# melspectrum007/audio-visual-speech-enhancement

Hardware: AMD Instinct MI355X
Metric: clips/sec (STFT+CNN forward) on 200-ms@16kHz segments, 1/2/4/8 MI355X (higher is better)
Workload: dtype fp32_split

## Files before the change

### audio-visual-speech-enhancement_amd/csrc/avse_common.h

```cpp
#pragma once
#include <hip/hip_runtime.h>
#include <stdint.h>
#include <string>

#include "forward_plan.h"
#include "ragged_geom.h"

typedef __bf16 bf16_t;
typedef __bf16 bf16x8 __attribute__((ext_vector_type(8)));
typedef _Float16 f16x8 __attribute__((ext_vector_type(8)));
typedef _Float16 f16x4 __attribute__((ext_vector_type(4)));
typedef float f32x4 __attribute__((ext_vector_type(4)));
typedef int i32x4 __attribute__((ext_vector_type(4)));

struct avse_ctx;

namespace avse {

void set_error(const std::string& msg);

int ctx_device_index(const struct ::avse_ctx* c);

int ensure_lds_attr(const void* fn, int bytes);

// ... 154 lines not shown
constexpr int kConvSplit = 2, kConvSplitPairs = 3;
int launch_conv(const ConvArgs& a, int dtype, hipStream_t s);

int launch_conv_win(const ConvArgs& a, const int2* htaps, hipStream_t s);

struct DecTailArgs {
    const bf16_t* in;
    float* out;
    int N;
    const bf16_t* w4;
    const float* sc4;
    const float* sh4;
    int nt4, kpad4;
    int pt4, pl4, rows4, pitch4;
    int dy4, dx4, nx4;
    const bf16_t* w5;
    const float* sc5;
    const float* sh5;
    int nt5[4], kpad5[4];
    int dy5[4], dx5[4], nx5[4];
    long long woff5[4];
    int pt5, pl5, rows5, pitch5;
    const float* w6;
    float b6;
    unsigned* range_flag;
    unsigned range_bit;
    int four_products;
};
bool dec_tail_supported(const DecTailArgs& a);
bool dec_tail_s16_supported(const DecTailArgs& a);
int launch_dec_tail_s16(const DecTailArgs& a, hipStream_t s);

struct AudEncArgs {
    const float* mel;
    bf16_t* out;
    long long out_clip_stride;
    int N;
    const bf16_t* w1;
    const bf16_t* w2;
    const bf16_t* w3;
    const bf16_t* w4;
    const bf16_t* w5;
    const float* sc[5];
    const float* sh[5];
};
bool aud_enc_supported(const AudEncArgs& a);

struct DecHeadArgs {
    const bf16_t* in;
    long long in_clip_stride;
    bf16_t* out;
    long long out_clip_stride;
    int N;
    const bf16_t* w1;
    const bf16_t* w2;
    const bf16_t* w3;
    const float* sc[3];
    const float* sh[3];
};
bool dec_head_supported(const DecHeadArgs& a);
int launch_dec_head(const DecHeadArgs& a, hipStream_t s);

struct GemmArgs {
    const bf16_t* a;
    long long lda;
    const bf16_t* w;
    int M, N, kpad;
    const float* scale;
    const float* shift;
    int act;
    bf16_t* out;
    long long ldo;
    int out_off;
    int ksplit;
    float* partial;
    int* counters;
    int split;
    int slabs_per_split;
    unsigned* range_flag;
    unsigned range_bit;
    int counters_cap;
    int four_products;
};
int launch_gemm(const GemmArgs& g, int mode, hipStream_t s);
int launch_aud_enc(const AudEncArgs& a, hipStream_t s);
int launch_dec_tail(const DecTailArgs& a, hipStream_t s);

enum HaloOut { OUT_BF16 = 0, OUT_S16 = 1, OUT_F32 = 2 };

struct HaloArgs {
    int variant;
    const void* in;
    const float* video;
    const float* vmean;
    const float* vstd;
    void* out;
    const void* w;
    const float* scale;
    const float* shift;
    int N, Hc, Wc, Ci, Co;
    long long out_clip_stride;
    int out_pix_stride;
    int out_c_off;
    int mfma32;
    int no_planar;
    int split;
    int out_mode;
    unsigned long long* prof;
    unsigned* range_flag;
    unsigned range_bit, range_in_bit;
    int video_u8;
};

int launch_conv_stream(const HaloArgs& a, hipStream_t s);
int launch_conv_v1r(const HaloArgs& a, hipStream_t s);
int launch_video_prep(const void* video, int video_u8, const float* mean, const float* stdv, void* out, int64_t N,
                      int F, int dtype, hipStream_t s);
int launch_audio_prep(const float* audio, void* out, int64_t npix, int dtype, hipStream_t s);
int launch_aconv1_split(const float* in, const float* w, const float* scale, const float* shift, void* out, int64_t N,
                        int H, int W, int Ho, int Wo, int KH, int KW, int S, int pt, int pl, int Co, unsigned* range_flag,
                        unsigned range_bit, unsigned range_in_bit, hipStream_t s);
int launch_out_conv(const void* in, const float* w64, float bias, float* out, int64_t npix, int dtype,
                    hipStream_t s);
int launch_broadcast_row(const void* src, void* dst, int64_t rows, int64_t row_bytes, int64_t stride_bytes,
                         hipStream_t s);
int launch_video_normalize(float* video, int64_t S, int H, int W, int F, const float* mean,
                           const float* stdv, hipStream_t s);
int launch_mse(const float* a, const float* b, int64_t n, float* loss, float* partial, hipStream_t s);

size_t mix_pairs_scratch_bytes(int64_t n_pairs);
int launch_mix_pairs(const int16_t* speech, const int64_t* speech_off, const int16_t* noise, const int64_t* noise_off,
                     const double* snr_lin, int64_t n_pairs, int64_t L, float* rows, double* mix64, double* factor,
                     void* scratch, hipStream_t s);
constexpr int kVideoStatsMaxF = 8;
size_t video_stats_scratch_bytes(int64_t S, int H, int W);
int launch_video_stats(const float* video, int64_t S, int H, int W, int F, float* mean, float* stdv, void* scratch,
                       hipStream_t s);
int launch_video_stats_u8(const uint8_t* video, int64_t S, int H, int W, int F, float* mean, float* stdv, void* scratch,
                          hipStream_t s);

struct EvalDev {
    const double* taps;
    const double* W;
    const double* twid;
    const double* segw;
    const int* bands;
    int up, down, H;
    int win, skip;
    int stoi;
    int64_t cap;
    const double* ptaps;
    int ms;
};
size_t eval_pairs_scratch_bytes(int64_t n_pairs, const EvalDev& t);
int launch_eval_pairs(const float* ref, const float* deg, const int64_t* off, int64_t n_pairs, const EvalDev& t,
                      double* metrics, void* scratch, hipStream_t s);

}
```

### audio-visual-speech-enhancement_amd/csrc/capi.hip

```cpp
#include <algorithm>
#include <cmath>
#include <cstdlib>
#include <cstring>
#include <mutex>
#include <set>

#include "ctx.h"
#include "eval_tables.h"
#include "spec_tables.h"

namespace avse {
static thread_local std::string g_err;
void set_error(const std::string& msg) { g_err = msg; }

int ensure_lds_attr(const void* fn, int bytes) {
    static std::mutex mu;
    static std::set<std::pair<const void*, int>> done;
    int dev = 0;
    AVSE_HIP_CHECK(hipGetDevice(&dev));
    std::lock_guard<std::mutex> lock(mu);
    if (done.count({fn, dev})) return 0;
    AVSE_HIP_CHECK(hipFuncSetAttribute(fn, hipFuncAttributeMaxDynamicSharedMemorySize, bytes));
    done.insert({fn, dev});
    return 0;
}

int fail(int code, const std::string& msg) {
    set_error(msg);
    return code;
}

int ctx_device_index(const avse_ctx* c) { return c->device; }
}

using namespace avse;

static_assert(sizeof(Cplx) == sizeof(float2) && offsetof(Cplx, im) == offsetof(float2, y), "Cplx must match float2");
static_assert(sizeof(MelBin) == sizeof(float4) && offsetof(MelBin, j0) == offsetof(float4, z), "MelBin must match float4");

struct OptionName {
    const char* name;
    const char* env;
    int Options::*field;
};
const OptionName kOptionNames[] = {
    {"no_gemm", "AVSE_NO_GEMM", &Options::no_gemm},
    {"no_audenc", "AVSE_NO_AUDENC", &Options::no_audenc},
    {"no_dechead", "AVSE_NO_DECHEAD", &Options::no_dechead},
    {"no_dectail", "AVSE_NO_DECTAIL", &Options::no_dectail},
    {"unfused_tail", "AVSE_UNFUSED_TAIL", &Options::unfused_tail},
    {"no_halo", "AVSE_NO_HALO", &Options::no_halo},
    {"mfma32", "AVSE_MFMA32", &Options::mfma32},
    {"serial", "AVSE_SERIAL", &Options::serial},
    {"graph", "AVSE_GRAPH", &Options::graph},
    {"gemm_ksplit_cap", "AVSE_GEMM_KSPLIT", &Options::gemm_ksplit_cap},
    {"dense_istft", "AVSE_DENSE_ISTFT", &Options::dense_istft},
    {"no_act_scale", "AVSE_NO_ACT_SCALE", &Options::no_act_scale},
    {"no_win", "AVSE_NO_WIN", &Options::no_win},
    {"no_v1p", "AVSE_NO_V1P", &Options::no_v1p},
    {"no_a1valu", "AVSE_NO_A1VALU", &Options::no_a1valu},
    {"no_planar", "AVSE_NO_PLANAR", &Options::no_planar},
    {"four_products", "AVSE_FOUR_PRODUCTS", &Options::four_products},
    {"side_prio", "AVSE_SIDE_PRIO", &Options::side_prio},
};

namespace {

const OptionName* find_option(const char* name) {
    for (const OptionName& o : kOptionNames)
        if (std::strcmp(o.name, name) == 0) return &o;
    return nullptr;
}

int upload_ragged(avse_ctx* c, const RaggedGeom& g, hipStream_t s, RaggedDev* d) {
    const size_t ub = sizeof(RaggedUtt) * g.utt.size(), ib = sizeof(RaggedItem) * g.items.size();
    const size_t need = ub + ib;
    hipStreamCaptureStatus cs = hipStreamCaptureStatusNone;
    if (s) AVSE_HIP_CHECK(hipStreamIsCapturing(s, &cs));
    const bool capturing = cs != hipStreamCaptureStatusNone;
    if (int rc = grow(c->prep, need, s, "preprocess scratch")) return rc;
    if (!capturing && c->ragged_done) AVSE_HIP_CHECK(hipEventSynchronize(c->ragged_done));
    if (int rc = grow(c->ragged_host, need, s, "ragged tables")) return rc;
    if (!c->ragged_done) AVSE_HIP_CHECK(hipEventCreateWithFlags(&c->ragged_done, hipEventDisableTiming));
    std::memcpy(c->ragged_host, g.utt.data(), ub);
    std::memcpy(c->ragged_host + ub, g.items.data(), ib);
    AVSE_HIP_CHECK(hipMemcpyAsync(c->prep, c->ragged_host, need, hipMemcpyHostToDevice, s));
    if (!capturing) AVSE_HIP_CHECK(hipEventRecord(c->ragged_done, s));
    d->utt = reinterpret_cast<const RaggedUtt*>(c->prep.p.get());
    d->items = reinterpret_cast<const RaggedItem*>(c->prep + ub);
    d->n_utt = (int)g.utt.size();
    d->n_items = (int)g.items.size();
    return 0;
}

template <typename D, typename T>
int table_to_device(const std::vector<T>& h, Owned<D>& out) {
    static_assert(sizeof(D) == sizeof(T), "element layout");
    AVSE_HIP_CHECK(out.alloc(sizeof(T) * h.size()));
    AVSE_HIP_CHECK(hipMemcpy(out, h.data(), sizeof(T) * h.size(), hipMemcpyHostToDevice));
    return 0;
}

int ensure_spec_tables(avse_ctx* c, int sr, int n_fft, int n_mels, double fmin, double fmax) {
    return build_spec_tables(c->spec, sr, n_fft, n_mels, fmin, fmax);
}

int ensure_istft_tables(avse_ctx* c, int sr, int n_fft, int n_mels, double fmin, double fmax) {
    return build_istft_tables(c->istft, sr, n_fft, n_mels, fmin, fmax);
}

int ensure_eval_tables(avse_ctx* c, int sr, bool any_rate, hipStream_t s, const EvalTables** out) {
    int up, down;
    eval_ratio(sr, &up, &down);
    const bool big = any_rate && std::max(up, down) > kEvalMaxRatio;
    for (const EvalTables& have : c->eval)
        if (have.sr == sr && have.big == big) {
            *out = &have;
            return 0;
        }
    if (int rc = not_capturing(s, "the tables of this sample rate would be built while the stream is being captured: run "
                                  "one call with this rate before the capture"))
        return rc;
    EvalTables& t = c->eval[c->eval_next];
    c->eval_next = (c->eval_next + 1) % 4;
    *out = &t;
    t = EvalTables();
    const int win = seg_snr_window(sr);
    const bool stoi = big || std::max(up, down) <= kEvalMaxRatio;
    const std::vector<double> taps = stoi ? resample_taps(up, down) : resample_taps(1, 1);
    if (big) {
        if (int rc = table_to_device(resample_taps_by_phase(taps, up), t.ptaps)) return rc;
    } else {
        if (int rc = table_to_device(taps, t.taps)) return rc;
    }
    if (int rc = table_to_device(hann_inner(kStoiFrame), t.W)) return rc;
    if (int rc = table_to_device(stoi_twiddle(), t.twid)) return rc;
    if (int rc = table_to_device(hann_inner(win), t.segw)) return rc;
    if (int rc = table_to_device(stoi_bands(), t.bands)) return rc;
    t.up = up; t.down = down; t.H = ((int)taps.size() - 1) / 2; t.win = win;
    t.sr = sr;
    t.big = big;
    return 0;
}

int spec_check(bool pointers, int64_t n_utt, const int64_t* n_samples, int sr, int n_fft, int hop, int n_mels, int pad_mode,
// ... 380 lines not shown
```

### audio-visual-speech-enhancement_amd/csrc/forward.hip

```cpp
#include <algorithm>
#include <cstdio>
#include <cstring>

#include "ctx.h"

using namespace avse;

namespace {

HaloArgs halo_args(const GpuLayer& G, const void* in, const void* video, int video_dtype, const float* vmean,
                   const float* vstd, void* out, long long out_clip_stride, int out_pix_stride, int out_c_off, int64_t N,
                   const Options& opt) {
    HaloArgs a;
    std::memset(&a, 0, sizeof(a));
    a.variant = G.halo;
    a.in = in;
    a.video = reinterpret_cast<const float*>(video);
    a.video_u8 = video_dtype == AVSE_VIDEO_U8;
    a.vmean = vmean;
    a.vstd = vstd;
    a.out = out;
    a.w = G.w_halo;
    a.mfma32 = opt.mfma32;
    a.no_planar = opt.no_planar;
// ... 90 lines not shown
    a.Wq = G.wq;
    a.sy = (L.kind == CONV) ? L.sh : 1;
    a.sx = (L.kind == CONV) ? L.sw : 1;
    a.oys = (L.kind == DECONV) ? L.sh : 1;
    a.oxs = (L.kind == DECONV) ? L.sw : 1;
    a.Ho = G.ho;
    a.Wo = G.wo;
    a.Co = L.cout;
    a.out_clip_stride = out_clip_stride;
    a.out_pix_stride = out_pix_stride;
    a.out_c_off = out_c_off;
    a.pool = L.pool ? 1 : 0;
    a.act = 1;
    a.nphase = G.nphase;
    a.ksplit = 1;
    for (int p = 0; p < G.nphase; ++p) a.ph[p] = G.ph[p];
    return a;
}

int ensure_arena(avse_ctx* c, int64_t clips, int dtype, const ArenaShape& a, hipStream_t s) {
    const size_t need = std::max(arena_bytes(clips, dtype, c->opt, nullptr, a), arena_bytes(1, dtype, c->opt, nullptr, a));
    return grow(c->arena, need, s, "forward scratch", "call avse_ctx_reserve_weights(ctx, weights, max_clips) before the capture");
}

struct Run {
    avse_ctx* c;
    const avse_weights* W;
    const Options& opt;
    const NetPlan& P;
    hipStream_t s;
    hipEvent_t* ev;
    const int dt;
    const bool split;
    const int gdt;
    const int cdt;
    const bool use_gemm;
    int stage = 0;

    Run(avse_ctx* c_, const avse_weights* W_, hipStream_t s_, hipEvent_t* ev_)
        : c(c_), W(W_), opt(c_->opt), P(W_->shape.plan), s(s_), ev(ev_), dt(W_->dtype), split(dt == AVSE_F32_SPLIT),
          gdt(dt == AVSE_BF16 ? AVSE_BF16 : AVSE_F32), cdt(split ? kConvSplit : gdt),
          use_gemm((dt == AVSE_BF16 || split) && !opt.no_gemm) {}

    const GpuLayer& L(int i) const { return W->layers[i]; }
    size_t es() const { return dt == AVSE_BF16 ? 2 : 4; }

    int mark() {
        if (ev) AVSE_HIP_CHECK(hipEventRecord(ev[stage], s));
        ++stage;
        return 0;
    }
    int mark(int n) {
        for (int k = 0; k < n; ++k)
            if (int rc = mark()) return rc;
        return 0;
    }

    int pairs(ConvArgs& a, bool in_pairs, bool out_pairs, int li, unsigned* rflag) const {
        if (!split) return gdt;
        a.range_flag = rflag;
        a.range_bit = 1u << li;
        a.range_in_bit = li == 0 ? kRangeAudioIn : kRangeVideoIn;
        if (in_pairs) {
            a.Ci *= 2;
            a.in_clip_stride *= 2;
            for (int p = 0; p < a.nphase; ++p) {
                a.ph[p].kpad *= 2;
                a.ph[p].w_off *= 2;
            }
        }
        if (out_pairs) {
            a.out_s16 = 1;
            a.out_clip_stride *= 2;
            a.out_pix_stride *= 2;
            a.out_c_off *= 2;
        }
        return in_pairs ? kConvSplitPairs : kConvSplit;
    }

    int conv(const ConvArgs& a, int dti, const GpuLayer& G, hipStream_t st) const {
        if (split && dti == kConvSplitPairs && !opt.no_win) {
            const int rw = launch_conv_win(a, G.htaps, st);
            if (rw != -1) return rw;
        }
        return launch_conv(a, split ? dti : cdt, st);
    }

    int gemm_layer(int li, const void* in, long long lda, void* out, long long ldo, int out_pix_stride, int out_off,
                   int64_t n, size_t part_off, unsigned* rflag) const {
        const GpuLayer& G = L(li);
        const SplitPlan sp = split_plan(W->shape.split[li - kSplitFirst], n, dt, opt);
        float* partial = reinterpret_cast<float*>(c->arena + part_off);
        const int mode = li == kSplitFirst ? 1 : 0;
        if (use_gemm && (mode == 0 || W->v6_gemm_shape)) {
            GemmArgs g;
            std::memset(&g, 0, sizeof(g));
            g.a = reinterpret_cast<const bf16_t*>(in);
            g.w = reinterpret_cast<const bf16_t*>(G.w);
            g.out = reinterpret_cast<bf16_t*>(out);
            g.lda = split ? 2 * lda : lda;
            g.ldo = split ? 2 * ldo : ldo;
            g.out_off = split ? 2 * out_off : out_off;
            g.M = (int)(mode == 1 ? n * 16 : n); g.N = G.def.cout; g.kpad = G.ph[0].kpad;
            g.scale = G.scale; g.shift = G.shift; g.act = 1;
            g.ksplit = sp.gemm.ksplit; g.slabs_per_split = sp.gemm.slabs; g.partial = partial;
            g.counters = c->gemm_counters; g.counters_cap = kGemmCounters;
            g.split = split; g.four_products = opt.four_products;
            if (split) { g.range_flag = rflag; g.range_bit = 1u << li; }
            const int rc = launch_gemm(g, mode, s);
            if (rc != -1) return rc;
        }
        ConvArgs a = conv_args(G, in, lda, out, ldo, out_pix_stride, out_off, n);
        a.ksplit = sp.conv.ksplit; a.ksplit_slabs = sp.conv.slabs; a.partial = partial;
        const int dti = pairs(a, true, true, li, rflag);
        return launch_conv(a, split ? dti : cdt, s);
    }

    int video_encoder(const void* vid, int vid_dt, const float* vm, const float* vs, int64_t n, const size_t* o,
                      void* cat, unsigned* rflag, bool record) {
        const long long CAT = P.cat, AEMB = P.aemb;
        auto vb = [&](int b) { return (void*)(c->arena + o[b]); };
        const int v_in[6] = {B_VIN, B_V1, B_V2, B_V3, B_V4, B_V5};
        int rc;
        if (L(5).halo == HALO_NONE &&
            (rc = launch_video_prep(vid, vid_dt == AVSE_VIDEO_U8, vm, vs, vb(B_VIN), n, P.F, gdt, s)))
            return rc;
        for (int i = 0; i < 6; ++i) {
            const GpuLayer& G = L(5 + i);
            const long long in_cs = (long long)G.def.hin * G.def.win * (i == 0 ? G.cin_pad : G.def.cin);
            if (G.halo != HALO_NONE) {
                HaloArgs h = (i < 5) ? halo_args(G, vb(v_in[i]), vid, vid_dt, vm, vs, vb(v_in[i + 1]),
                                                 (long long)G.ho * G.wo * G.def.cout, G.def.cout, 0, n, opt)
                                     : halo_args(G, vb(v_in[i]), vid, vid_dt, vm, vs, cat, CAT, G.def.cout, AEMB, n, opt);
                if (split) {
                    h.split = 1;
                    h.range_flag = rflag;
                    h.range_bit = 1u << (5 + i);
                    h.range_in_bit = kRangeVideoIn;
                    if (G.halo != HALO_V1 && G.halo != HALO_V1P) h.Ci = 2 * G.def.cin;
                    h.out_mode = OUT_S16;
                    h.out_clip_stride *= 2;
                    h.out_pix_stride *= 2;
                    h.out_c_off *= 2;
                }
                rc = G.halo == HALO_V1 || G.halo == HALO_V1P ? launch_conv_v1r(h, s) : launch_conv_stream(h, s);
            } else if (i == 5) {
                rc = gemm_layer(5 + i, vb(v_in[i]), in_cs, cat, CAT, G.def.cout, AEMB, n, o[B_COUNT], rflag);
            } else {
                ConvArgs a = conv_args(G, vb(v_in[i]), in_cs, vb(v_in[i + 1]), (long long)G.ho * G.wo * G.def.cout, G.def.cout, 0, n);
                const int dti = pairs(a, i > 0, true, 5 + i, rflag);
                rc = launch_conv(a, split ? dti : cdt, s);
            }
            if (rc || (record && (rc = mark()))) return rc;
        }
        return 0;
    }

    int zero_video_embedding() {
        if (W->vzero_emb.load(std::memory_order_acquire)) return 0;
        std::lock_guard<std::mutex> lk(W->vzero_mu);
        if (W->vzero_emb.load(std::memory_order_relaxed)) return 0;
        if (int rc = not_capturing(s, "the all-zero-video embedding must be computed before graph capture")) return rc;
        if (!c->zero_video) {
            AVSE_HIP_CHECK(c->zero_video.alloc(sizeof(float) * 128 * 128 * 8));
            AVSE_HIP_CHECK(hipMemsetAsync(c->zero_video, 0, sizeof(float) * 128 * 128 * 8, s));
        }
// ... 346 lines not shown
```

### audio-visual-speech-enhancement_amd/csrc/gemm.hip

```cpp
#include <algorithm>
#include <cstdlib>

#include "avse_common.h"

namespace avse {
namespace {

constexpr float LRELU = 0.3f;
constexpr int kOOB = 0x7fffff00;
constexpr int NT = 512;
constexpr int SLAB = 16384;
constexpr int GRP = 4 * SLAB;
constexpr int LDS_BYTES = 2 * GRP;

__device__ __forceinline__ __amdgpu_buffer_rsrc_t make_rsrc(const void* base, long long bytes) {
    const int nrec = bytes > kOOB ? kOOB : (bytes < 0 ? 0 : (int)bytes);
    return __builtin_amdgcn_make_buffer_rsrc(const_cast<void*>(base), (short)0, nrec, 0x00020000);
}
__device__ __forceinline__ int wsw(int row) { return 2 * ((row >> 2) & 1); }
__device__ __forceinline__ i32x4 lds16(const char* p) { return *reinterpret_cast<const i32x4*>(p); }

template <int MODE, int ABL = 0, bool S16 = false, bool PR = S16>
__global__ __launch_bounds__(NT, 1) void k_gemm(GemmArgs g) {
    extern __shared__ __attribute__((aligned(1024))) char lds[];
    __shared__ int last_flag;
    const int tid = threadIdx.x, lane = tid & 63;
    const int w = __builtin_amdgcn_readfirstlane(tid >> 6);
    const int r16 = lane & 15, kg = lane >> 4;
    const int wm = w >> 2, wn = w & 3;
    const int m0 = blockIdx.x * 128, n0 = blockIdx.y * 128, z = blockIdx.z;
    constexpr int KB = S16 ? 4 : 2;
    const int nslab_all = g.kpad * KB / 64;
    const int sps = S16 && g.slabs_per_split > 0 ? g.slabs_per_split : (nslab_all + g.ksplit - 1) / g.ksplit;
    const int s_begin = z * sps, nsl = min(nslab_all, s_begin + sps) - s_begin;

    const int lrow = tid >> 2, part = tid & 3;
    const int ldst = lrow * 64 + ((part ^ wsw(lrow)) << 4);
    const __amdgpu_buffer_rsrc_t rsW = make_rsrc(g.w, (long long)g.N * g.kpad * KB);
    const int wvoff = (n0 + lrow < g.N) ? (n0 + lrow) * g.kpad * KB + part * 16 : kOOB;
    constexpr int PIXB = 512 * KB, CPT = PIXB / 64;
    __amdgpu_buffer_rsrc_t rsA;
    int avoff = kOOB, py = 0, px = 0;
    if constexpr (MODE == 0) {
        rsA = make_rsrc(g.a, (long long)g.M * g.lda * 2);
        if (m0 + lrow < g.M) avoff = (m0 + lrow) * (int)g.lda * 2 + part * 16;
    } else {
        const int m = m0 + lrow, clip = m >> 4, p = m & 15, q = p >> 2, e = p & 3;
        py = 2 * (q >> 1) + (e >> 1);
        px = 2 * (q & 1) + (e & 1);
        rsA = make_rsrc(g.a, (long long)(g.M >> 4) * g.lda * 2);
        if (m < g.M) avoff = clip * (int)g.lda * 2 + (py * 4 + px) * PIXB + part * 16;
    }
    auto load = [&](int s, i32x4& va, i32x4& vw) {
        if constexpr ((ABL & 2) != 0) {
            va = vw = (i32x4){s, 0, 0, 0};
            return;
        }
        const int sa = s_begin + (s < nsl ? s : 0);
        const bool pad = S16 && s >= nsl;
        vw = __builtin_amdgcn_raw_buffer_load_b128(rsW, pad ? kOOB : wvoff, sa * 64, 0);
        if constexpr (MODE == 0) {
            va = __builtin_amdgcn_raw_buffer_load_b128(rsA, pad ? kOOB : avoff, sa * 64, 0);
        } else {
            const int tap = sa / CPT, c = sa % CPT, dy = tap / 3 - 1, dx = tap - 3 * (tap / 3) - 1;
            const bool ok = (unsigned)(py + dy) < 4u && (unsigned)(px + dx) < 4u && avoff != kOOB && !pad;
            va = __builtin_amdgcn_raw_buffer_load_b128(rsA, ok ? avoff + (dy * 4 + dx) * PIXB : kOOB, c * 64, 0);
        }
    };
    auto store = [&](int s, const i32x4& va, const i32x4& vw) {
        char* const d = lds + ((s >> 2) & 1) * GRP + (s & 3) * SLAB + ldst;
        *reinterpret_cast<i32x4*>(d) = va;
        *reinterpret_cast<i32x4*>(d + 8192) = vw;
    };
    const int afr = (64 * wm + r16) * 64 + ((kg ^ wsw(r16)) << 4);
    const int bfr = 8192 + (32 * wn + r16) * 64 + (((S16 ? kg & 1 : kg) ^ wsw(r16)) << 4);
    const int bfl = 8192 + (32 * wn + r16) * 64 + (((2 + (kg & 1)) ^ wsw(r16)) << 4);
    const int pso = (kg >> 1) * SLAB;
    const int pah = pso + (64 * wm + r16) * 64 + (((kg & 1) ^ wsw(r16)) << 4);
    const int pal = pso + (64 * wm + r16) * 64 + (((2 + (kg & 1)) ^ wsw(r16)) << 4);
    i32x4 fa[2][4], fb[2][2], fl[2][2], fal[2][4];
    auto read_pair = [&](int s, int buf) {
        const char* const b = lds + ((s >> 2) & 1) * GRP + (s & 3) * SLAB;
#pragma unroll
        for (int i = 0; i < 4; ++i) fa[buf][i] = lds16(b + pah + 1024 * i);
#pragma unroll
        for (int i = 0; i < 4; ++i) fal[buf][i] = lds16(b + pal + 1024 * i);
#pragma unroll
        for (int j = 0; j < 2; ++j) fb[buf][j] = lds16(b + pso + bfr + 1024 * j);
#pragma unroll
        for (int j = 0; j < 2; ++j) fl[buf][j] = lds16(b + pso + bfl + 1024 * j);
    };
    auto read = [&](int s, int buf) {
        const char* const b = lds + ((s >> 2) & 1) * GRP + (s & 3) * SLAB;
#pragma unroll
        for (int i = 0; i < 4; ++i) fa[buf][i] = lds16(b + afr + 1024 * i);
#pragma unroll
        for (int j = 0; j < 2; ++j) fb[buf][j] = lds16(b + bfr + 1024 * j);
        if constexpr (S16) {
#pragma unroll
            for (int j = 0; j < 2; ++j) fl[buf][j] = lds16(b + bfl + 1024 * j);
        }
    };
    f32x4 acc[4][2], blk[4][2];
#pragma unroll
    for (int i = 0; i < 4; ++i) acc[i][0] = acc[i][1] = blk[i][0] = blk[i][1] = (f32x4){0.f, 0.f, 0.f, 0.f};
    float esc[2], esh[2];
#pragma unroll
    for (int j = 0; j < 2; ++j) {
        const int n = n0 + 32 * wn + 16 * j + r16;
        esc[j] = n < g.N ? g.scale[n] : 0.f;
        esh[j] = n < g.N ? g.shift[n] : 0.f;
    }

    i32x4 ra[4], rw[4];
    {
        i32x4 a0[4], w0[4];
#pragma unroll
        for (int s = 0; s < 4; ++s) load(s, a0[s], w0[s]);
#pragma unroll
        for (int s = 0; s < 4; ++s) load(s + 4, ra[s], rw[s]);
#pragma unroll
        for (int s = 0; s < 4; ++s) store(s, a0[s], w0[s]);
    }
    __syncthreads();
    if constexpr (S16 && PR) read_pair(0, 0);
    else read(0, 0);
    if constexpr (S16 && PR) {
        const int npad8 = (nsl + kFp32Block - 1) & ~(kFp32Block - 1);
        for (int s0 = 0; s0 < npad8; s0 += kFp32Block) {
#pragma unroll
            for (int p = 0; p < kFp32Block / 2; ++p) {
                const int s = s0 + 2 * p, q0 = (2 * p) & 3, q1 = (2 * p + 1) & 3;
                __builtin_amdgcn_sched_barrier(0);
                store(s + 4, ra[q0], rw[q0]);
                load(s + 8, ra[q0], rw[q0]);
                store(s + 5, ra[q1], rw[q1]);
                load(s + 9, ra[q1], rw[q1]);
                if (p & 1) __syncthreads();
                read_pair(s + 2, (p + 1) & 1);
                __builtin_amdgcn_sched_barrier(0);
                if constexpr ((ABL & 4) != 0) {
#pragma unroll
                    for (int i = 0; i < 4; ++i)
                        blk[i][0][0] += __builtin_bit_cast(float, fa[p & 1][i][0] ^ fal[p & 1][i][3] ^ fb[p & 1][i & 1][1] ^
                                                                      fl[p & 1][i & 1][2]);
                    continue;
                }
#pragma unroll
                for (int h = 0; h < 3; ++h)
#pragma unroll
                    for (int i = 0; i < 4; ++i)
#pragma unroll
                        for (int j = 0; j < 2; ++j)
                            blk[i][j] = __builtin_amdgcn_mfma_f32_16x16x32_f16(
                                __builtin_bit_cast(f16x8, h == 1 ? fal[p & 1][i] : fa[p & 1][i]),
                                __builtin_bit_cast(f16x8, h == 2 ? fl[p & 1][j] : fb[p & 1][j]), blk[i][j], 0, 0, 0);
            }
#pragma unroll
            for (int i = 0; i < 4; ++i)
#pragma unroll
                for (int j = 0; j < 2; ++j) {
                    acc[i][j] += blk[i][j];
                    blk[i][j] = (f32x4){0.f, 0.f, 0.f, 0.f};
                }
        }
    } else if constexpr (S16) {
        const int npad8 = (nsl + kFp32Block - 1) & ~(kFp32Block - 1);
        for (int s0 = 0; s0 < npad8; s0 += kFp32Block) {
#pragma unroll
            for (int q = 0; q < kFp32Block; ++q) {
                const int s = s0 + q;
                __builtin_amdgcn_sched_barrier(0);
                store(s + 4, ra[q & 3], rw[q & 3]);
                load(s + 8, ra[q & 3], rw[q & 3]);
                if ((q & 3) == 3) __syncthreads();
                read(s + 1, (q + 1) & 1);
                __builtin_amdgcn_sched_barrier(0);
                if constexpr ((ABL & 4) != 0) {
#pragma unroll
                    for (int i = 0; i < 4; ++i)
                        blk[i][0][0] += __builtin_bit_cast(float, fa[q & 1][i][0] ^ fb[q & 1][i & 1][1] ^ fl[q & 1][i & 1][2]);
                    continue;
                }
#pragma unroll
                for (int h = 0; h < 2; ++h)
#pragma unroll
                    for (int i = 0; i < 4; ++i)
#pragma unroll
                        for (int j = 0; j < 2; ++j)
                            blk[i][j] = __builtin_amdgcn_mfma_f32_16x16x32_f16(
                                __builtin_bit_cast(f16x8, fa[q & 1][i]), __builtin_bit_cast(f16x8, h ? fl[q & 1][j] : fb[q & 1][j]),
                                blk[i][j], 0, 0, 0);
            }
#pragma unroll
            for (int i = 0; i < 4; ++i)
#pragma unroll
                for (int j = 0; j < 2; ++j) {
                    acc[i][j] += blk[i][j];
                    blk[i][j] = (f32x4){0.f, 0.f, 0.f, 0.f};
                }
        }
    }
    const int npad = S16 ? 0 : (nsl + 3) & ~3;
    for (int s0 = 0; s0 < npad; s0 += 4) {
#pragma unroll
        for (int q = 0; q < 4; ++q) {
            const int s = s0 + q;
            __builtin_amdgcn_sched_barrier(0);
            store(s + 4, ra[q], rw[q]);
            load(s + 8, ra[q], rw[q]);
            if (q == 3) __syncthreads();
            if (s + 1 < nsl) read(s + 1, (q + 1) & 1);
            __builtin_amdgcn_sched_barrier(0);
            if (s < nsl) {
#pragma unroll
                for (int i = 0; i < 4; ++i)
#pragma unroll
                    for (int j = 0; j < 2; ++j)
                        acc[i][j] = __builtin_amdgcn_mfma_f32_16x16x32_bf16(__builtin_bit_cast(bf16x8, fa[q & 1][i]),
                                                                             __builtin_bit_cast(bf16x8, fb[q & 1][j]),
                                                                             acc[i][j], 0, 0, 0);
            }
        }
    }

    if (g.ksplit > 1) {
        const int tile = blockIdx.y * gridDim.x + blockIdx.x;
        const __amdgpu_buffer_rsrc_t rsP = make_rsrc(g.partial + (size_t)tile * g.ksplit * 8 * NT * 4,
                                                     (long long)g.ksplit * 8 * NT * 16);
#pragma unroll
        for (int i = 0; i < 4; ++i)
#pragma unroll
            for (int j = 0; j < 2; ++j)
                __builtin_amdgcn_raw_buffer_store_b128(__builtin_bit_cast(i32x4, acc[i][j]), rsP,
                                                       ((z * 8 + i * 2 + j) * NT + tid) * 16, 0, 16 );
        asm volatile("s_waitcnt vmcnt(0)" ::: "memory");
        __syncthreads();
        if (tid == 0)
            last_flag = __hip_atomic_fetch_add(g.counters + tile, 1, __ATOMIC_RELAXED, __HIP_MEMORY_SCOPE_AGENT) == g.ksplit - 1;
        __syncthreads();
        if (!last_flag) return;
#pragma unroll
        for (int i = 0; i < 4; ++i)
#pragma unroll
            for (int j = 0; j < 2; ++j) acc[i][j] = (f32x4){0.f, 0.f, 0.f, 0.f};
        for (int zz = 0; zz < ((ABL & 1) ? 0 : g.ksplit); ++zz)
#pragma unroll
            for (int i = 0; i < 4; ++i)
#pragma unroll
                for (int j = 0; j < 2; ++j)
                    acc[i][j] += __builtin_bit_cast(f32x4, __builtin_amdgcn_raw_buffer_load_b128(
                                                               rsP, ((zz * 8 + i * 2 + j) * NT + tid) * 16, 0, 16 ));
        if (tid == 0) g.counters[tile] = 0;
    }

    bool bad = false;
    auto put = [&](long long base, int n, float v) {
        if constexpr (S16) {
            const _Float16 h = (_Float16)v, l = (_Float16)(v - (float)h);
            bad |= pair_out_of_range(v);
            unsigned short* o = reinterpret_cast<unsigned short*>(g.out) + base + (n >> 4) * 32 + (n & 15);
            o[0] = __builtin_bit_cast(unsigned short, h);
            o[16] = __builtin_bit_cast(unsigned short, l);
        } else {
            g.out[base + n] = (bf16_t)v;
        }
    };
#pragma unroll
    for (int j = 0; j < 2; ++j) {
        const int n = n0 + 32 * wn + 16 * j + r16;
        if (n >= g.N) continue;
        const float sc = esc[j], sh = esh[j];
#pragma unroll
        for (int i = 0; i < 4; ++i) {
            const int mb = m0 + 64 * wm + 16 * i + 4 * kg;
            if (mb >= g.M) continue;
            if constexpr (MODE == 0) {
#pragma unroll
                for (int e = 0; e < 4; ++e) {
                    if (mb + e >= g.M) continue;
                    float v = acc[i][j][e] * sc + sh;
                    if (g.act) v = v >= 0.f ? v : LRELU * v;
                    put((long long)(mb + e) * g.ldo + g.out_off, n, v);
                }
            } else {
                float v = fmaxf(fmaxf(acc[i][j][0] * sc + sh, acc[i][j][1] * sc + sh),
                                fmaxf(acc[i][j][2] * sc + sh, acc[i][j][3] * sc + sh));
                if (g.act) v = v >= 0.f ? v : LRELU * v;
                const int clip = mb >> 4, q = (mb & 15) >> 2;
                put((long long)clip * g.ldo + g.out_off + q * g.N * (S16 ? 2 : 1), n, v);
            }
        }
    }
    if constexpr (S16) range_report(g.range_flag, g.range_bit, bad);
}

}

int launch_gemm(const GemmArgs& g, int mode, hipStream_t s) {
    const bool s16 = g.split != 0;
#ifndef AVSE_GEMM_ABL
#define AVSE_GEMM_ABL 0
#endif
    const bool pr = s16 && !g.four_products;
    const void* kf = mode == 0 ? (pr    ? (const void*)k_gemm<0, AVSE_GEMM_ABL, true, true>
                                  : s16 ? (const void*)k_gemm<0, AVSE_GEMM_ABL, true, false>
                                        : (const void*)k_gemm<0>)
                               : (pr    ? (const void*)k_gemm<1, AVSE_GEMM_ABL, true, true>
                                  : s16 ? (const void*)k_gemm<1, AVSE_GEMM_ABL, true, false>
                                        : (const void*)k_gemm<1>);
    if (int rc = ensure_lds_attr(kf, LDS_BYTES)) return rc;
    const int kq = s16 ? 16 : 32;
    const int nslab = g.kpad / kq;
    const bool s16_bad = s16 && (g.N % 16 || (g.ksplit > 1 && (g.slabs_per_split <= 0 || g.slabs_per_split % kFp32Block ||
                                                               (nslab + g.slabs_per_split - 1) / g.slabs_per_split != g.ksplit)));
    if (g.kpad % kq || g.M <= 0 || g.N <= 0 || g.ksplit < 1 || (g.ksplit > 1 && (!g.partial || !g.counters)) ||
        (mode == 1 && (g.M % 16 || g.kpad != 9 * 512)) || s16_bad) {
        set_error("gemm: bad arguments");
        return 3;
    }
    if (!gemm_tickets_fit(g.M, g.N, g.ksplit, g.counters_cap)) return -1;
    const dim3 grid((g.M + 127) / 128, (g.N + 127) / 128, g.ksplit);
    hipLaunchKernelGGL(reinterpret_cast<void (*)(GemmArgs)>(const_cast<void*>(kf)), grid, dim3(NT), LDS_BYTES, s, g);
    AVSE_HIP_CHECK(hipGetLastError());
    return 0;
}

}
```

### audio-visual-speech-enhancement_amd/csrc/layer_geom.h

```cpp
#pragma once
#include <utility>
#include <vector>

#include "netplan.h"

namespace avse {

constexpr int MAX_TAPS = 25;
constexpr int MAX_PHASES = 4;

struct ConvPhase {
    int py, px;
    int ntaps;
    int kpad;
    long long w_off;
    int tap_off;
};

struct Tap {
    int dy, dx;
};

inline long long kidx(const LayerDef& L, int ky, int kx, int ci, int co) {
    if (L.kind == DENSE) return (long long)ci * L.cout + co;
// ... 76 lines not shown
inline LayerGeom layer_geom(const LayerDef& L) {
    LayerGeom g;
    g.cin_pad = g.cp = pad8(L.cin);
    g.rows = L.cout;
    g.red = L.cin;
    if (L.kind == DECONV) {
        g.pt = (L.kh > L.sh ? L.kh - L.sh : 0) / 2;
        g.pl = (L.kw > L.sw ? L.kw - L.sw : 0) / 2;
        g.hq = L.hin;
        g.wq = L.win;
        g.hz = L.hin * L.sh;
        g.wz = L.win * L.sw;
        set_phases(g, subpixel_phases(L.kh, L.sh, g.pt), subpixel_phases(L.kw, L.sw, g.pl));
    } else {
        g.pt = same_pad_before(L.hin, L.kh, L.sh);
        g.pl = same_pad_before(L.win, L.kw, L.sw);
        g.hq = g.hz = same_out(L.hin, L.sh);
        g.wq = g.wz = same_out(L.win, L.sw);
        set_phases(g, gather_taps(L.kh, g.pt), gather_taps(L.kw, g.pl));
    }
    g.ho = L.pool ? g.hz / 2 : g.hz;
    g.wo = L.pool ? g.wz / 2 : g.wz;
    return g;
}

struct DgradGeom : PhaseSet {
    int ci = 0;
    int hq = 1, wq = 1;
    int sy = 1, sx = 1;
    int oys = 1, oxs = 1;
};

inline DgradGeom dgrad_geom(const LayerDef& L) {
    const LayerGeom f = layer_geom(L);
    DgradGeom g;
    g.dgrad = true;
    g.ci = g.cp = pad8(L.cout);
    g.rows = L.cin;
    g.red = L.cout;
    if (L.kind == DECONV) {
        g.hq = L.hin;
        g.wq = L.win;
        g.sy = L.sh;
        g.sx = L.sw;
        set_phases(g, gather_taps(L.kh, f.pt), gather_taps(L.kw, f.pl));
        return g;
    }
    if (L.hin % L.sh || L.win % L.sw) {
        g.status = GEOM_DGRAD_STRIDE;
        return g;
    }
    g.hq = L.hin / L.sh;
    g.wq = L.win / L.sw;
    g.oys = L.sh;
    g.oxs = L.sw;
    set_phases(g, subpixel_phases(L.kh, L.sh, f.pt), subpixel_phases(L.kw, L.sw, f.pl));
    for (int p = 0; p < g.nphase && g.status == GEOM_OK; ++p)
        if (g.ph[p].ntaps == 0) g.status = GEOM_DGRAD_EMPTY_PHASE;
    return g;
}

inline std::vector<int> gather_map(const LayerDef& L, const PhaseSet& g) {
    std::vector<int> m((size_t)g.w_elems, -1);
    for (int p = 0; p < g.nphase; ++p)
        for (int n = 0; n < g.rows; ++n) {
            int* row = m.data() + (size_t)g.ph[p].w_off + (size_t)n * g.ph[p].kpad;
            for (size_t j = 0; j < g.kyx[p].size(); ++j) {
                const int ky = g.kyx[p][j].first, kx = g.kyx[p][j].second;
                const long long k0 = g.dgrad ? kidx(L, ky, kx, n, 0) : kidx(L, ky, kx, 0, n);
                const long long dk = (g.dgrad ? kidx(L, ky, kx, n, 1) : kidx(L, ky, kx, 1, n)) - k0;
                for (int c = 0; c < g.red; ++c) row[j * g.cp + c] = (int)(k0 + c * dk);
            }
        }
    return m;
}

constexpr int kFp32Block = 8;

constexpr int kGemmCounters = 8192;
inline bool gemm_tickets_fit(long long M, long long N, int ksplit, long long counters) {
    return ksplit <= 1 || ((M + 127) / 128) * ((N + 127) / 128) <= counters;
}

}
```

### audio-visual-speech-enhancement_amd/csrc/options.h

```cpp
#pragma once

namespace avse {

struct Options {
    int no_gemm = 0;
    int no_audenc = 0;
    int no_dechead = 0;
    int no_dectail = 0;
    int unfused_tail = 0;
    int no_halo = 0;
    int mfma32 = 0;
    int serial = 0;
    int graph = 0;
    int gemm_ksplit_cap = 0;
    int dense_istft = 0;
    int no_act_scale = 0;
    int no_win = 0;
    int no_v1p = 0;
    int no_a1valu = 0;
    int no_planar = 0;
    int four_products = 0;
    int side_prio = 0;
};

enum HaloVariant { HALO_NONE = -1, HALO_V1 = 0, HALO_K5 = 1, HALO_K3_16 = 2, HALO_K3_8 = 3, HALO_V1P = 4 };

}
```

Baseline: 81900.

## Route split-pair conv and deconv layers through implicit-GEMM MFMA kernel

Adds a new MODE 2 to the tiled GEMM kernel that does implicit-GEMM convolution. It gathers input pixels per tap through buffer loads, runs one grid z-slice per sub-pixel phase, and scatters the results to strided output positions with fused scale, shift and leaky ReLU. The conv dispatcher tries this path for split-pair layers whose shapes are on a whitelist, after the windowed kernel declines. It is meant to replace the generic direct-conv kernel with the MFMA-tiled GEMM pipeline. The costs are per-row tap address computation, no k-split for these layers, and the risk of poor occupancy on small layers.

Result: no change. 81990, median of 2 (+0.1%).

```diff
diff --git a/audio-visual-speech-enhancement_amd/csrc/avse_common.h b/audio-visual-speech-enhancement_amd/csrc/avse_common.h
--- a/audio-visual-speech-enhancement_amd/csrc/avse_common.h
+++ b/audio-visual-speech-enhancement_amd/csrc/avse_common.h
@@ -260,7 +260,11 @@
     int counters_cap;
     int four_products;
 };
+struct GemmConvArgs : GemmArgs {
+    GemmConvGeom cv;
+};
 int launch_gemm(const GemmArgs& g, int mode, hipStream_t s);
+int launch_gemm_conv(const ConvArgs& a, const int2* htaps, int four_products, hipStream_t s);
 int launch_aud_enc(const AudEncArgs& a, hipStream_t s);
 int launch_dec_tail(const DecTailArgs& a, hipStream_t s);
 
diff --git a/audio-visual-speech-enhancement_amd/csrc/capi.hip b/audio-visual-speech-enhancement_amd/csrc/capi.hip
--- a/audio-visual-speech-enhancement_amd/csrc/capi.hip
+++ b/audio-visual-speech-enhancement_amd/csrc/capi.hip
@@ -61,6 +61,7 @@
     {"no_a1valu", "AVSE_NO_A1VALU", &Options::no_a1valu},
     {"no_planar", "AVSE_NO_PLANAR", &Options::no_planar},
     {"four_products", "AVSE_FOUR_PRODUCTS", &Options::four_products},
+    {"no_gemm_conv", "AVSE_NO_GEMM_CONV", &Options::no_gemm_conv},
     {"side_prio", "AVSE_SIDE_PRIO", &Options::side_prio},
 };
 
diff --git a/audio-visual-speech-enhancement_amd/csrc/forward.hip b/audio-visual-speech-enhancement_amd/csrc/forward.hip
--- a/audio-visual-speech-enhancement_amd/csrc/forward.hip
+++ b/audio-visual-speech-enhancement_amd/csrc/forward.hip
@@ -196,6 +196,10 @@
         if (split && dti == kConvSplitPairs && !opt.no_win) {
             const int rw = launch_conv_win(a, G.htaps, st);
             if (rw != -1) return rw;
+        }
+        if (split && dti == kConvSplitPairs && !(opt.no_gemm_conv & (G.def.kind == DECONV ? 1 : 2))) {
+            const int rg = launch_gemm_conv(a, G.htaps, opt.four_products, st);
+            if (rg != -1) return rg;
         }
         return launch_conv(a, split ? dti : cdt, st);
     }
diff --git a/audio-visual-speech-enhancement_amd/csrc/gemm.hip b/audio-visual-speech-enhancement_amd/csrc/gemm.hip
--- a/audio-visual-speech-enhancement_amd/csrc/gemm.hip
+++ b/audio-visual-speech-enhancement_amd/csrc/gemm.hip
@@ -1,5 +1,7 @@
 #include <algorithm>
 #include <cstdlib>
+#include <cstring>
+#include <type_traits>
 
 #include "avse_common.h"
 
@@ -21,29 +23,43 @@
 __device__ __forceinline__ i32x4 lds16(const char* p) { return *reinterpret_cast<const i32x4*>(p); }
 
 template <int MODE, int ABL = 0, bool S16 = false, bool PR = S16>
-__global__ __launch_bounds__(NT, 1) void k_gemm(GemmArgs g) {
+__global__ __launch_bounds__(NT, 1) void k_gemm(std::conditional_t<MODE == 2, GemmConvArgs, GemmArgs> g) {
     extern __shared__ __attribute__((aligned(1024))) char lds[];
     __shared__ int last_flag;
     const int tid = threadIdx.x, lane = tid & 63;
     const int w = __builtin_amdgcn_readfirstlane(tid >> 6);
     const int r16 = lane & 15, kg = lane >> 4;
     const int wm = w >> 2, wn = w & 3;
-    const int m0 = blockIdx.x * 128, n0 = blockIdx.y * 128, z = blockIdx.z;
+    const int m0 = blockIdx.x * 128, n0 = blockIdx.y * 128, z = MODE == 2 ? 0 : blockIdx.z;
+    const int phase = MODE == 2 ? blockIdx.z : 0;
     constexpr int KB = S16 ? 4 : 2;
-    const int nslab_all = g.kpad * KB / 64;
+    int kpad = g.kpad;
+    if constexpr (MODE == 2) kpad = g.cv.kpad[phase];
+    const int nslab_all = kpad * KB / 64;
     const int sps = S16 && g.slabs_per_split > 0 ? g.slabs_per_split : (nslab_all + g.ksplit - 1) / g.ksplit;
     const int s_begin = z * sps, nsl = min(nslab_all, s_begin + sps) - s_begin;
 
     const int lrow = tid >> 2, part = tid & 3;
     const int ldst = lrow * 64 + ((part ^ wsw(lrow)) << 4);
-    const __amdgpu_buffer_rsrc_t rsW = make_rsrc(g.w, (long long)g.N * g.kpad * KB);
-    const int wvoff = (n0 + lrow < g.N) ? (n0 + lrow) * g.kpad * KB + part * 16 : kOOB;
+    const void* wbase = g.w;
+    if constexpr (MODE == 2) wbase = reinterpret_cast<const char*>(g.w) + g.cv.w_off[phase];
+    const __amdgpu_buffer_rsrc_t rsW = make_rsrc(wbase, (long long)g.N * kpad * KB);
+    const int wvoff = (n0 + lrow < g.N) ? (n0 + lrow) * kpad * KB + part * 16 : kOOB;
     constexpr int PIXB = 512 * KB, CPT = PIXB / 64;
     __amdgpu_buffer_rsrc_t rsA;
     int avoff = kOOB, py = 0, px = 0;
+    int cur_tap = -1, atap = kOOB;
     if constexpr (MODE == 0) {
         rsA = make_rsrc(g.a, (long long)g.M * g.lda * 2);
         if (m0 + lrow < g.M) avoff = (m0 + lrow) * (int)g.lda * 2 + part * 16;
+    } else if constexpr (MODE == 2) {
+        const int hw = g.cv.Hq * g.cv.Wq, clip0 = m0 / hw, m = m0 + lrow;
+        const GemmConvRow r = gemm_conv_row(m < g.M ? m : m0, g.cv.Hq, g.cv.Wq);
+        py = r.qy;
+        px = r.qx;
+        rsA = make_rsrc(reinterpret_cast<const char*>(g.a) + clip0 * g.cv.in_clip_bytes,
+                        (g.M / hw - clip0) * g.cv.in_clip_bytes);
+        if (m < g.M) avoff = (r.clip - clip0) * (int)g.cv.in_clip_bytes + part * 16;
     } else {
         const int m = m0 + lrow, clip = m >> 4, p = m & 15, q = p >> 2, e = p & 3;
         py = 2 * (q >> 1) + (e >> 1);
@@ -61,6 +77,16 @@
         vw = __builtin_amdgcn_raw_buffer_load_b128(rsW, pad ? kOOB : wvoff, sa * 64, 0);
         if constexpr (MODE == 0) {
             va = __builtin_amdgcn_raw_buffer_load_b128(rsA, pad ? kOOB : avoff, sa * 64, 0);
+        } else if constexpr (MODE == 2) {
+            const int tap = __builtin_amdgcn_readfirstlane(gemm_conv_slab_tap(s, g.cv.cpt_log2));
+            const int c = gemm_conv_slab_chunk(s, g.cv.cpt_log2);
+            if (tap != cur_tap) {
+                cur_tap = tap;
+                const int t = g.cv.taps[phase][tap < kGemmConvTaps ? tap : kGemmConvTaps - 1];
+                const int pix = gemm_conv_in_pixel(g.cv, py, px, gemm_conv_tap_dy(t), gemm_conv_tap_dx(t));
+                atap = tap < g.cv.ntaps[phase] && pix >= 0 && avoff != kOOB ? avoff + pix : kOOB;
+            }
+            va = __builtin_amdgcn_raw_buffer_load_b128(rsA, atap, c * 64, 0);
         } else {
             const int tap = sa / CPT, c = sa % CPT, dy = tap / 3 - 1, dx = tap - 3 * (tap / 3) - 1;
             const bool ok = (unsigned)(py + dy) < 4u && (unsigned)(px + dx) < 4u && avoff != kOOB && !pad;
@@ -224,7 +250,7 @@
         }
     }
 
-    if (g.ksplit > 1) {
+    if (MODE != 2 && g.ksplit > 1) {
         const int tile = blockIdx.y * gridDim.x + blockIdx.x;
         const __amdgpu_buffer_rsrc_t rsP = make_rsrc(g.partial + (size_t)tile * g.ksplit * 8 * NT * 4,
                                                      (long long)g.ksplit * 8 * NT * 16);
@@ -266,6 +292,20 @@
             g.out[base + n] = (bf16_t)v;
         }
     };
+    long long orow[MODE == 2 ? 4 : 1][4];
+    (void)orow;
+    if constexpr (MODE == 2) {
+#pragma unroll
+        for (int i = 0; i < 4; ++i) {
+            const int mb = m0 + 64 * wm + 16 * i + 4 * kg;
+            GemmConvRow r = gemm_conv_row(mb, g.cv.Hq, g.cv.Wq);
+#pragma unroll
+            for (int e = 0; e < 4; ++e) {
+                orow[i][e] = mb + e < g.M ? gemm_conv_out_offset(g.cv, phase, r) : -1;
+                r = gemm_conv_next_row(r, g.cv.Hq, g.cv.Wq);
+            }
+        }
+    }
 #pragma unroll
     for (int j = 0; j < 2; ++j) {
         const int n = n0 + 32 * wn + 16 * j + r16;
@@ -275,7 +315,15 @@
         for (int i = 0; i < 4; ++i) {
             const int mb = m0 + 64 * wm + 16 * i + 4 * kg;
             if (mb >= g.M) continue;
-            if constexpr (MODE == 0) {
+            if constexpr (MODE == 2) {
+#pragma unroll
+                for (int e = 0; e < 4; ++e) {
+                    if (orow[i][e] < 0) continue;
+                    float v = acc[i][j][e] * sc + sh;
+                    if (g.act) v = v >= 0.f ? v : LRELU * v;
+                    put(orow[i][e], n, v);
+                }
+            } else if constexpr (MODE == 0) {
 #pragma unroll
                 for (int e = 0; e < 4; ++e) {
                     if (mb + e >= g.M) continue;
@@ -326,4 +374,72 @@
     return 0;
 }
 
-}
+namespace {
+
+struct GemmConvShape {
+    int Ci, Co, Hi, nphase, ntaps0, sy, sx, oys, oxs;
+};
+constexpr GemmConvShape kGemmConvAccept[] = {
+    {64, 128, 40, 1, 16, 2, 2, 1, 1},
+    {128, 128, 20, 1, 4, 2, 1, 1, 1},
+    {128, 128, 10, 1, 4, 2, 1, 1, 1},
+    {128, 128, 5, 2, 2, 1, 1, 2, 1},
+    {128, 128, 10, 2, 2, 1, 1, 2, 1},
+    {128, 128, 20, 4, 4, 1, 1, 2, 2},
+};
+
+}
+
+int launch_gemm_conv(const ConvArgs& a, const int2* htaps, int four_products, hipStream_t s) {
+    if (!a.out_s16 || a.Co % 128 || a.pool || a.fuse_w || a.ksplit > 1 || a.nphase < 1 || a.nphase > MAX_PHASES) return -1;
+    const int pix_bytes = a.Ci * 2;
+    if (pix_bytes <= 0 || pix_bytes % 64) return -1;
+    const int cpt = pix_bytes / 64;
+    if (cpt & (cpt - 1)) return -1;
+    bool listed = false;
+    for (const GemmConvShape& t : kGemmConvAccept)
+        listed |= a.Ci == 2 * t.Ci && a.Co == t.Co && a.Hi == t.Hi && a.nphase == t.nphase && a.ph[0].ntaps == t.ntaps0 &&
+                  a.sy == t.sy && a.sx == t.sx && a.oys == t.oys && a.oxs == t.oxs;
+    if (!listed) return -1;
+    const long long hw = (long long)a.Hq * a.Wq, M = a.N * hw, clip_bytes = a.in_clip_stride * 2;
+    if (hw <= 0 || M <= 0 || M > 0x7fffff00LL || clip_bytes * (128 / hw + 2) >= kOOB) return -1;
+    GemmConvArgs g;
+    std::memset(&g, 0, sizeof(g));
+    GemmConvGeom& cv = g.cv;
+    cv.Hq = a.Hq; cv.Wq = a.Wq; cv.Hi = a.Hi; cv.Wi = a.Wi; cv.sy = a.sy; cv.sx = a.sx;
+    cv.oys = a.oys; cv.oxs = a.oxs; cv.Wo = a.Wo;
+    cv.cpt_log2 = __builtin_ctz(cpt);
+    cv.pix_bytes = pix_bytes;
+    cv.in_clip_bytes = clip_bytes;
+    cv.out_clip_stride = a.out_clip_stride; cv.out_pix_stride = a.out_pix_stride; cv.out_c_off = a.out_c_off;
+    for (int p = 0; p < a.nphase; ++p) {
+        const ConvPhase& ph = a.ph[p];
+        if (ph.ntaps < 1 || ph.ntaps > kGemmConvTaps || ph.kpad * 2 != ph.ntaps * cpt * 64 ||
+            (long long)a.Co * ph.kpad * 2 >= kOOB)
+            return -1;
+        cv.py[p] = ph.py; cv.px[p] = ph.px; cv.ntaps[p] = ph.ntaps;
+        cv.kpad[p] = ph.kpad / 2;
+        cv.w_off[p] = ph.w_off * 2;
+        for (int t = 0; t < ph.ntaps; ++t) {
+            const int2 d = htaps[ph.tap_off + t];
+            if (d.x < -32768 || d.x > 32767 || d.y < -32768 || d.y > 32767) return -1;
+            cv.taps[p][t] = gemm_conv_pack_tap(d.x, d.y);
+        }
+    }
+    g.a = reinterpret_cast<const bf16_t*>(a.in);
+    g.w = reinterpret_cast<const bf16_t*>(a.w);
+    g.out = reinterpret_cast<bf16_t*>(a.out);
+    g.M = (int)M; g.N = a.Co;
+    g.scale = a.scale; g.shift = a.shift; g.act = a.act;
+    g.ksplit = 1; g.split = 1; g.four_products = four_products;
+    g.range_flag = a.range_flag; g.range_bit = a.range_bit;
+    const void* kf = four_products ? (const void*)k_gemm<2, AVSE_GEMM_ABL, true, false>
+                                   : (const void*)k_gemm<2, AVSE_GEMM_ABL, true, true>;
+    if (int rc = ensure_lds_attr(kf, LDS_BYTES)) return rc;
+    const dim3 grid((unsigned)((M + 127) / 128), a.Co / 128, a.nphase);
+    hipLaunchKernelGGL(reinterpret_cast<void (*)(GemmConvArgs)>(const_cast<void*>(kf)), grid, dim3(NT), LDS_BYTES, s, g);
+    AVSE_HIP_CHECK(hipGetLastError());
+    return 0;
+}
+
+}
diff --git a/audio-visual-speech-enhancement_amd/csrc/layer_geom.h b/audio-visual-speech-enhancement_amd/csrc/layer_geom.h
--- a/audio-visual-speech-enhancement_amd/csrc/layer_geom.h
+++ b/audio-visual-speech-enhancement_amd/csrc/layer_geom.h
@@ -182,4 +182,59 @@
     return ksplit <= 1 || ((M + 127) / 128) * ((N + 127) / 128) <= counters;
 }
 
-}
+constexpr int kGemmConvTaps = 16;
+struct GemmConvGeom {
+    int Hq, Wq;
+    int Hi, Wi;
+    int sy, sx;
+    int oys, oxs, Wo;
+    int cpt_log2;
+    int pix_bytes;
+    long long in_clip_bytes;
+    long long out_clip_stride;
+    int out_pix_stride, out_c_off;
+    int py[MAX_PHASES], px[MAX_PHASES], ntaps[MAX_PHASES];
+    int kpad[MAX_PHASES];
+    long long w_off[MAX_PHASES];
+    int taps[MAX_PHASES][kGemmConvTaps];
+};
+struct GemmConvRow {
+    int clip, qy, qx;
+};
+constexpr GemmConvRow gemm_conv_row(int m, int Hq, int Wq) {
+    const int hw = Hq * Wq, clip = m / hw, r = m - clip * hw, qy = r / Wq;
+    return GemmConvRow{clip, qy, r - qy * Wq};
+}
+constexpr int gemm_conv_slab_tap(int s, int cpt_log2) { return s >> cpt_log2; }
+constexpr int gemm_conv_slab_chunk(int s, int cpt_log2) { return s & ((1 << cpt_log2) - 1); }
+constexpr int gemm_conv_pack_tap(int dy, int dx) { return (dy & 0xffff) | (int)((unsigned)dx << 16); }
+constexpr int gemm_conv_tap_dy(int t) { return (int)(short)(t & 0xffff); }
+constexpr int gemm_conv_tap_dx(int t) { return t >> 16; }
+constexpr int gemm_conv_in_pixel(const GemmConvGeom& g, int qy, int qx, int dy, int dx) {
+    const int iy = qy * g.sy + dy, ix = qx * g.sx + dx;
+    return (unsigned)iy < (unsigned)g.Hi && (unsigned)ix < (unsigned)g.Wi ? (iy * g.Wi + ix) * g.pix_bytes : -1;
+}
+constexpr long long gemm_conv_out_offset(const GemmConvGeom& g, int p, const GemmConvRow& r) {
+    return r.clip * g.out_clip_stride +
+           (long long)((r.qy * g.oys + g.py[p]) * g.Wo + r.qx * g.oxs + g.px[p]) * g.out_pix_stride + g.out_c_off;
+}
+constexpr long long gemm_conv_a_offset(const GemmConvGeom& g, int M, int p, int m, int s) {
+    const int tap = gemm_conv_slab_tap(s, g.cpt_log2);
+    if (m >= M || tap >= g.ntaps[p]) return -1;
+    const GemmConvRow r = gemm_conv_row(m, g.Hq, g.Wq);
+    const int t = g.taps[p][tap];
+    const int pix = gemm_conv_in_pixel(g, r.qy, r.qx, gemm_conv_tap_dy(t), gemm_conv_tap_dx(t));
+    return pix < 0 ? -1 : r.clip * g.in_clip_bytes + pix + gemm_conv_slab_chunk(s, g.cpt_log2) * 64;
+}
+constexpr GemmConvRow gemm_conv_next_row(GemmConvRow r, int Hq, int Wq) {
+    if (++r.qx == Wq) {
+        r.qx = 0;
+        if (++r.qy == Hq) {
+            r.qy = 0;
+            ++r.clip;
+        }
+    }
+    return r;
+}
+
+}
diff --git a/audio-visual-speech-enhancement_amd/csrc/options.h b/audio-visual-speech-enhancement_amd/csrc/options.h
--- a/audio-visual-speech-enhancement_amd/csrc/options.h
+++ b/audio-visual-speech-enhancement_amd/csrc/options.h
@@ -20,6 +20,7 @@
     int no_a1valu = 0;
     int no_planar = 0;
     int four_products = 0;
+    int no_gemm_conv = 0;
     int side_prio = 0;
 };
 
```
